# tayloraswift/swift-png

Measured on AMD Instinct MI355X. Metric: decoded_mpixels_per_s, higher is better.
Workload: dtype u8

## Files before the change

swift_png_amd/csrc/pinflate2.hip:

```cpp
#include "common.hpp"
#include <type_traits>
#include <cstddef>
#include "huffman.hpp"

namespace spng {

#ifdef SPNG_EMU
#define AS_GLOBAL
#else
#define AS_GLOBAL __attribute__((address_space(1)))
#endif
__device__ __forceinline__ uint32_t mul24(uint32_t a, uint32_t b)
{
#ifdef SPNG_EMU
    return (a & 0xffffffu) * (b & 0xffffffu);
#else
    uint32_t r;
    asm("v_mul_u32_u24 %0, %1, %2" : "=v"(r) : "v"(a), "v"(b));
    return r;
#endif
}
typedef uint32_t v4u __attribute__((vector_size(16)));
struct __attribute__((packed)) PV4 { v4u v; };
typedef uint8_t AS_GLOBAL g8;
typedef uint16_t AS_GLOBAL g16;
typedef uint32_t AS_GLOBAL g32;
typedef PV4 AS_GLOBAL gPV4;
typedef uint32_t v2u __attribute__((vector_size(8)));
struct __attribute__((packed)) PV2 { v2u v; };
typedef PV2 AS_GLOBAL gPV2;

#ifdef SPNG_NO_HINTS
#define RARE(c) (c)
#else
#define RARE(c) __builtin_expect((c), 0)
#endif
static constexpr int LB = 9, DB = 8, MB = 7;
#ifndef SPNG_SDW_MAX
#define SPNG_SDW_MAX 9
#endif
static constexpr int SDW_MAX = SPNG_SDW_MAX;
static constexpr int STAGE2_DW = SDW_MAX * 64 + 16;
static constexpr uint32_t PAGE_SHIFT = 16;
static constexpr uint32_t PAGE_UNITS = 1u << (PAGE_SHIFT - 4);
static constexpr uint64_t NONE2 = ~0ull;
static constexpr uint32_t TK_NULL = 0xffffu;

__device__ __forceinline__ uint32_t tk_m0(uint32_t run, uint32_t dist) { return 0x8000u | ((dist - 1) & 63) << 8 | (run - 3); }
__device__ __forceinline__ uint32_t tk_m1(uint32_t dist) { return 0xC000u | (dist - 1) >> 6; }

struct DPool { uint8_t *base; uint32_t *next; uint32_t pages, pad; };

#ifdef SPNG_D_PROF
#define DP_ARG , uint64_t *dp
#define DP_PASS , dp
#define DP(k) do { const uint64_t now_ = __builtin_readcyclecounter(); dp[k] += now_ - dp[31]; dp[31] = now_; } while (0)
#define DPN(k, v) (dp[k] += (v))
#define HP_ARG , uint64_t *dp = nullptr
#define HP(k) do { if (dp) DP(k); } while (0)
#else
#define DP_ARG
#define DP_PASS
#define DP(k)
#define DPN(k, v)
#define HP_ARG
#define HP(k)
#endif

#if defined(SPNG_EMU) && defined(SPNG_EMU_COV)
static long g_cov[13];
#define COV(k) __atomic_fetch_add(&g_cov[k], 1, __ATOMIC_RELAXED)
#else
#define COV(k) ((void)0)
#endif

static constexpr uint32_t EXT = 480;

enum { C_LIT = 0, C_EOB = 1, C_REF = 2, C_BAD = 3, C_LIT2 = 6, C_LINK = 7 };
__device__ __forceinline__ uint32_t lit_entry2(uint32_t sym, uint32_t len)
{
    if (sym < 256) return len | C_LIT << 5 | len << 8 | sym << 16;
    if (sym == 256) return len | C_EOB << 5 | len << 8;
    uint32_t base, cx;
    if (sym < 265) { base = sym - 254; cx = 0; }
    else if (sym < 285) { cx = (sym - 261) >> 2; base = ((4 + ((sym - 265) & 3)) << cx) + 3; }
    else if (sym == 285) { base = 258; cx = 0; }
    else { base = 0; cx = 0; }
    return (len + cx) | (base ? C_REF : C_BAD) << 5 | len << 8 | cx << 12 | base << 16;
}
__device__ __forceinline__ uint32_t dist_entry2(uint32_t sym, uint32_t len)
{
    uint32_t base, ox;
    if (sym < 4) { base = sym + 1; ox = 0; }
    else if (sym < 30) { ox = (sym >> 1) - 1; base = ((2 + (sym & 1)) << ox) + 1; }
    else { base = 0; ox = 0; }
    return (len + ox) | (base ? 0u : 32u) | len << 8 | ox << 12 | base << 16;
}
static constexpr uint32_t DIST_UNDEF = 1 | 32;

struct DLds {
    uint32_t lit[1 << LB];
    uint32_t dist[1 << DB];
    uint32_t ext[EXT];
    uint32_t stage[STAGE2_DW];
    union {
        struct {
            uint8_t  lens[512];
            uint32_t clut[1 << MB];
            uint32_t hb[6][16];
            uint32_t cl[32];
            uint16_t first[2][16];
            uint16_t codes[6][64];
        } h;
        struct {
            uint32_t ent[64];
            uint32_t vmap[SDW_MAX * 64];
            uint16_t flag[64], mpos[64];
        } c;
    };
};
static constexpr uint32_t QB = (uint32_t)offsetof(DLds, stage) * 8;
static_assert(QB % 32 == 0 && QB + (SDW_MAX * 64 + 3) * 32 + 64 < 65536, "biased positions: dword-aligned, 16 bits");
static_assert(offsetof(DLds, c.vmap) == offsetof(DLds, c.ent) + 256 && offsetof(DLds, c.flag) == offsetof(DLds, c.vmap) + SDW_MAX * 256,
              "round 1 reads ent as the row in front of vmap; round 0's empty OR behind a lane's last word lands in flag / mpos");

__device__ __forceinline__ v4u ld16(const g8 *src, uint64_t n, uint64_t off)
{
    v4u v = {0, 0, 0, 0};
    if (off + 16 <= n) v = ((const gPV4 *)(src + off))->v;
    else if (off < n) {
        uint32_t w[4] = {0, 0, 0, 0};
        for (int b = 0; b < 16; ++b) if (off + b < n) w[b >> 2] |= (uint32_t)src[off + b] << (8 * (b & 3));
        v[0] = w[0]; v[1] = w[1]; v[2] = w[2]; v[3] = w[3];
    }
    return v;
}
__device__ __forceinline__ void stage_bytes2(uint32_t *dst, const g8 *src, uint64_t n, uint64_t from, int dwords, int lane)
{
    for (int k = 0; k * 256 < dwords; ++k)
        if (k * 256 + lane * 4 < dwords) *(v4u *)(dst + k * 256 + lane * 4) = ld16(src, n, from + (uint64_t)k * 1024 + (uint64_t)lane * 16);
    WSYNC();
}
__device__ __forceinline__ void fetch2(const uint32_t *stage, uint32_t q, uint32_t &lo, uint32_t &hi)
{
    const uint32_t w = q >> 5;
    const uint32_t d0 = stage[w], d1 = stage[w + 1], d2 = stage[w + 2];
    lo = __builtin_amdgcn_alignbit(d1, d0, q);
    hi = __builtin_amdgcn_alignbit(d2, d1, q);
}
__device__ __forceinline__ uint32_t upeek32_2(const uint32_t *stage, uint32_t q)
{
    uint32_t lo, hi;
    fetch2(stage, q, lo, hi);
    return UNI(lo);
}
__device__ __forceinline__ uint64_t upeek64_2(const uint32_t *stage, uint32_t q)
{
    uint32_t lo, hi;
    fetch2(stage, q, lo, hi);
    return (uint64_t)UNI(hi) << 32 | UNI(lo);
}

struct Hdr2 {
    uint32_t type, bfinal;
    uint64_t payload;
    uint32_t stored;
    uint32_t minlen;
    uint32_t pairs;
};

template <int ROOT, int KIND>
__device__ __forceinline__ void place_symbol(uint32_t *lut, uint32_t sym, uint32_t my, uint32_t code)
{
    if (my <= (uint32_t)ROOT) lut[code << ((uint32_t)ROOT - my)] = KIND == 0 ? lit_entry2(sym, my) : dist_entry2(sym, my);
    else atomicMax(&lut[code >> (my - (uint32_t)ROOT)], my);
}
template <int ROOT, int KIND>
__device__ __forceinline__ void place_long(const uint32_t *lut, uint32_t *ext, uint32_t sym, uint32_t my, uint32_t code)
{
    if (my > (uint32_t)ROOT) {
        const uint32_t rev = __brev(code) >> (32 - my);
        const uint32_t link = lut[rev & ((1u << ROOT) - 1)];
        const uint32_t sub = (link >> 8) & 15, at = link >> 16;
        const uint32_t e = KIND == 0 ? lit_entry2(sym, my) : dist_entry2(sym, my);
        for (uint32_t j = rev >> ROOT; j < (1u << sub); j += 1u << (my - ROOT)) ext[at + j] = e;
    }
}
template <int ROOT>
__device__ __forceinline__ bool finish_root(uint32_t *lut, uint32_t &used, uint32_t cap, bool links, int lane)
{
    constexpr int PER = (1 << ROOT) / 64;
    uint32_t v[PER];
#pragma unroll
    for (int k = 0; k < PER; ++k) v[k] = lut[lane * PER + k];
#pragma unroll
    for (int k = 1; k < PER; ++k) v[k] = v[k] ? v[k] : v[k - 1];
    const unsigned long long have = __ballot(v[PER - 1] != 0) & ((1ull << lane) - 1);
    const uint32_t cin = (uint32_t)__shfl((int)v[PER - 1], have ? 63 - __clzll((long long)have) : 0, 64);
#pragma unroll
    for (int k = 0; k < PER; ++k) v[k] = v[k] ? v[k] : cin;
    if (links) {
        uint32_t need = 0;
#pragma unroll
        for (int k = 0; k < PER; ++k) need += (v[k] > (uint32_t)ROOT && v[k] <= 15) ? 1u << (v[k] - ROOT) : 0u;
        uint32_t tot;
        uint32_t at = used + wave_excl_scan(need, tot, lane);
        tot += used;
#ifdef SPNG_EMU_TRACE
        if (tot > cap && lane == 0) fprintf(stderr, "finish_root<%d>: need %u > cap %u\n", ROOT, tot, cap);
#endif
        if (tot > cap) return false;
        used = tot;
#pragma unroll
        for (int k = 0; k < PER; ++k)
            if (v[k] > (uint32_t)ROOT && v[k] <= 15) { const uint32_t sub = v[k] - ROOT; v[k] = C_LINK << 5 | sub << 8 | at << 16; at += 1u << sub; }
    }
    WSYNC();
#pragma unroll
    for (int k = 0; k < PER; ++k) lut[__brev((uint32_t)(lane * PER + k)) >> (32 - ROOT)] = v[k];
    return true;
}

__device__ __forceinline__ bool build_clut(DLds &s, uint32_t mylen, int lane)
{
    uint32_t cnt = 0, before = 0;
#pragma unroll
    for (uint32_t l = 1; l <= 7; ++l) {
        const unsigned long long m = __ballot(lane < 19 && mylen == l);
        cnt = (uint32_t)lane == l ? (uint32_t)__popcll(m) : cnt;
        before = mylen == l ? (uint32_t)__popcll(m & ((1ull << lane) - 1)) : before;
    }
    const uint32_t scaled = (lane >= 1 && lane <= 7) ? cnt << (7 - lane) : 0u;
    if (UNI(wave_sum(scaled)) != 128u) return false;
    const uint32_t first = ((row_scan(scaled) - scaled) >> (7 - (lane & 7))) & 127;
    if (lane < 16) s.h.cl[lane] = first;
    s.h.clut[lane] = 0; s.h.clut[64 + lane] = 0;
    WSYNC();
    if (lane < 19 && mylen)
        s.h.clut[(s.h.cl[mylen] + before) << (MB - mylen)] =
            mylen | (lane < 16 ? 0u : lane == 16 ? 2u : lane == 17 ? 3u : 7u) << 4 | (lane < 16 ? 1u : lane == 18 ? 11u : 3u) << 8 | (uint32_t)lane << 16;
    WSYNC();
    uint32_t none = 0;
    finish_root<MB>(s.h.clut, none, 0, false, lane);
    WSYNC();
    return true;
}

__device__ __attribute__((always_inline)) bool decode_lengths2(DLds &s, uint32_t &rel, uint32_t rel_end, uint32_t want, int lane)
{
    for (int i = lane; i < 128; i += 64) ((uint32_t *)s.h.lens)[i] = 0;
    uint32_t *list = s.lit;
    uint32_t ntok = 0, have = 0, p = rel;
    for (int window = 0; window < 80 && have < want; ++window) {
        if (p >= rel_end || p + 64 + 16 > 256u * 32) return false;
        const uint32_t q = p + (uint32_t)lane;
        const uint32_t w = q >> 5;
        const uint32_t bits = __builtin_amdgcn_alignbit(s.stage[w + 1], s.stage[w], q);
        const uint32_t e = s.h.clut[bits & ((1u << MB) - 1)];
        const uint32_t len = e & 15, sym = e >> 16, extra = (e >> 4) & 15;
        const uint32_t rep = ((e >> 8) & 0xff) + ((bits >> len) & ((1u << extra) - 1));
        const uint32_t nb = len + extra;
        uint32_t jn = nb, jr = rep;
        uint32_t jlo = lane < 32 ? 1u << lane : 0u, jhi = lane < 32 ? 0u : 1u << (lane - 32);
#pragma unroll
        for (int round = 0; round < 3; ++round) {
            const uint32_t tgt = (uint32_t)lane + jn;
            const uint32_t on = (uint32_t)__shfl((int)(jn | jr << 8), (int)(tgt & 63), 64);
            const uint32_t olo = (uint32_t)__shfl((int)jlo, (int)(tgt & 63), 64), ohi = (uint32_t)__shfl((int)jhi, (int)(tgt & 63), 64);
            if (tgt < 64) { jn += on & 0xff; jr += on >> 8; jlo |= olo; jhi |= ohi; }
        }
        unsigned long long mask = 0;
        uint32_t pp = 0;
        while (pp < 64) {
            mask |= (unsigned long long)(uint32_t)__builtin_amdgcn_readlane((int)jhi, (int)pp) << 32 | (uint32_t)__builtin_amdgcn_readlane((int)jlo, (int)pp);
            have += (uint32_t)__builtin_amdgcn_readlane((int)jr, (int)pp);
            pp += (uint32_t)__builtin_amdgcn_readlane((int)jn, (int)pp);
        }
        if ((mask >> lane) & 1) list[ntok + (uint32_t)__popcll(mask & ((1ull << lane) - 1))] = sym | rep << 8 | (q + nb) << 16;
        ntok += (uint32_t)__popcll(mask);
        p += pp;
    }
    if (have < want) return false;
    WSYNC();
    uint32_t prev = 0; bool prev_ok = false;
    have = 0;
    for (uint32_t b = 0; b < ntok; b += 64) {
        const bool is = b + (uint32_t)lane < ntok;
        const uint32_t t = is ? list[b + (uint32_t)lane] : 0u;
        const uint32_t sym = t & 0xff, r = (t >> 8) & 0xff;
        uint32_t tot;
        const uint32_t idx = have + wave_excl_scan(r, tot, lane);
        const uint32_t val = sym < 16 ? sym : 0u;
        const unsigned long long defm = __ballot(is && sym != 16);
        const unsigned long long below = defm & ((1ull << lane) - 1);
        const int pl = below ? 63 - __clzll((long long)below) : 0;
        const uint32_t pv = (uint32_t)__shfl((int)val, pl, 64);
        const uint32_t lastcur = below ? pv : prev;
        const bool ok = below ? true : prev_ok;
        const bool active = is && idx < want;
        const bool bad = active && (idx + r > want || (sym == 16 && !ok));
        if (active && !bad) {
            if (sym < 16) s.h.lens[idx] = (uint8_t)sym;
            else if (sym == 16) for (uint32_t k = 0; k < r; ++k) s.h.lens[idx + k] = (uint8_t)lastcur;
        }
        const unsigned long long endm = __ballot(active && idx + r == want);
        if (__ballot(bad)) return false;
        if (endm) {
            rel = (uint32_t)__builtin_amdgcn_readlane((int)(t >> 16), __ffsll((long long)endm) - 1);
            WSYNC();
            return rel <= rel_end;
        }
        have += tot;
        if (defm) { prev = (uint32_t)__shfl((int)val, 63 - __clzll((long long)defm), 64); prev_ok = true; }
    }
    return false;
}

__device__ __attribute__((always_inline)) bool build_tables2(DLds &s, uint32_t literals, uint32_t distances, uint32_t &minlen, uint32_t &pairs, int lane)
{
    uint32_t packed = 0;
#pragma unroll
    for (int k = 0; k < 5; ++k) { const uint32_t sym = (uint32_t)lane + 64u * k; packed |= (sym < literals ? (uint32_t)s.h.lens[sym] : 0u) << (4 * k); }
    packed |= ((uint32_t)lane < distances ? (uint32_t)s.h.lens[literals + lane] : 0u) << 20;
#define LL(k) ((packed >> (4 * (k))) & 15)
#define DL ((packed >> 20) & 15)
    for (int i = lane; i < 96; i += 64) (&s.h.hb[0][0])[i] = 0;
    WSYNC();
#pragma unroll
    for (int k = 0; k < 5; ++k) __hip_atomic_fetch_add(&s.h.hb[k][LL(k)], 1u, __ATOMIC_RELAXED, __HIP_MEMORY_SCOPE_WORKGROUP);
    __hip_atomic_fetch_add(&s.h.hb[5][DL], 1u, __ATOMIC_RELAXED, __HIP_MEMORY_SCOPE_WORKGROUP);
    const uint32_t dl = DL;
    const uint32_t dused = (uint32_t)__popcll(__ballot(dl != 0));
    const unsigned long long d1m = __ballot(dl == 1);
    WSYNC();
    const uint32_t L = (uint32_t)lane & 15;
    const bool isd = lane >= 16 && lane < 32;
    uint32_t c = 0;
// ... 8 lines not shown
    const uint32_t scaled = c << (15 - L);
    const uint32_t kraft = row_scan(scaled);
    const uint32_t klit = (uint32_t)__builtin_amdgcn_readlane((int)kraft, 15);
    const uint32_t kdist = (uint32_t)__builtin_amdgcn_readlane((int)kraft, 31);
    if (klit != 32768u) return false;
    const bool stub = dused == 0 || (dused == 1 && d1m != 0);
    if (!stub && kdist != 32768u) return false;
    if (lane < 32) s.h.first[isd ? 1 : 0][L] = (uint16_t)((kraft - scaled) >> (15 - L));
    {
        const unsigned long long nz = __ballot(lane < 16 && c != 0);
        minlen = (uint32_t)__ffsll((long long)nz) - 1;
    }
#pragma unroll
    for (int j = 0; j < (1 << LB) / 64; ++j) s.lit[j * 64 + lane] = 0;
#pragma unroll
    for (int j = 0; j < (1 << DB) / 64; ++j)
        s.dist[j * 64 + lane] = !stub ? 0u : (dused && !((j * 64 + lane) & 1)) ? dist_entry2((uint32_t)(__ffsll((long long)d1m) - 1), 1) : DIST_UNDEF;
    WSYNC();
#pragma unroll
    for (int k = 0; k < 5; ++k) {
        const uint32_t my = LL(k);
        unsigned long long same = ~0ull;
#pragma unroll
        for (int b = 0; b < 4; ++b) {
            const unsigned long long bk = __ballot((my >> b) & 1);
            same &= (my >> b) & 1 ? bk : ~bk;
        }
        if (my) {
            const uint32_t code = s.h.first[0][my] + s.h.hb[k][my] + (uint32_t)__popcll(same & ((1ull << lane) - 1));
            s.h.codes[k][lane] = (uint16_t)code;
            place_symbol<LB, 0>(s.lit, (uint32_t)lane + 64u * k, my, code);
        }
    }
    if (!stub) {
        const uint32_t my = dl;
        unsigned long long same = ~0ull;
#pragma unroll
        for (int b = 0; b < 4; ++b) {
            const unsigned long long bk = __ballot((my >> b) & 1);
            same &= (my >> b) & 1 ? bk : ~bk;
        }
        if (my) {
            const uint32_t code = s.h.first[1][my] + (uint32_t)__popcll(same & ((1ull << lane) - 1));
            s.h.codes[5][lane] = (uint16_t)code;
            place_symbol<DB, 1>(s.dist, (uint32_t)lane, my, code);
        }
    }
    WSYNC();
    const bool longl = __ballot(LL(0) > (uint32_t)LB || LL(1) > (uint32_t)LB || LL(2) > (uint32_t)LB || LL(3) > (uint32_t)LB || LL(4) > (uint32_t)LB) != 0;
    const bool longd = !stub && __ballot(dl > (uint32_t)DB) != 0;
    uint32_t used = 0;
    if (!UB(finish_root<LB>(s.lit, used, EXT, longl, lane))) return false;
    if (!stub) { if (!UB(finish_root<DB>(s.dist, used, EXT, longd, lane))) return false; }
    WSYNC();
    if (longl || longd) {
#pragma unroll
        for (int k = 0; k < 5; ++k) if (LL(k) > (uint32_t)LB) place_long<LB, 0>(s.lit, s.ext, (uint32_t)lane + 64u * k, LL(k), s.h.codes[k][lane]);
        if (!stub && dl > (uint32_t)DB) place_long<DB, 1>(s.dist, s.ext, (uint32_t)lane, dl, s.h.codes[5][lane]);
        WSYNC();
    }
#undef LL
#undef DL
    bool made = false;
    if (2 * minlen <= (uint32_t)LB)
#pragma unroll
    for (int k = 0; k < (1 << LB) / 64; ++k) {
        const uint32_t idx = (uint32_t)k * 64 + (uint32_t)lane;
        const uint32_t e = s.lit[idx];
        const uint32_t len0 = (e >> 8) & 15;
        if (((e >> 5) & 7) == C_LIT && len0 < (uint32_t)LB) {
            const uint32_t e2 = s.lit[idx >> len0];
            const uint32_t c2 = (e2 >> 5) & 7, len1 = (e2 >> 8) & 15;
            if ((c2 == C_LIT || c2 == C_LIT2) && len0 + len1 <= (uint32_t)LB) {
                s.lit[idx] = (len0 + len1) | C_LIT2 << 5 | len0 << 8 | (e & 0x00ff0000u) | (e2 & 0x00ff0000u) << 8;
                made = true;
            }
        }
    }
    pairs = __ballot(made) != 0 ? 1u : 0u;
    WSYNC();
    return true;
}

__device__ __attribute__((always_inline)) bool parse_header2(DLds &s, const g8 *src, uint64_t n, uint64_t pos, Hdr2 &h, int lane HP_ARG)
{
    const uint64_t total = n * 8;
    if (pos + 3 > total) return false;
    const uint64_t wbyte = (pos >> 5) << 2;
    stage_bytes2(s.stage, src, n, wbyte, 256, lane);
    HP(24);
    uint32_t rel = (uint32_t)(pos - wbyte * 8);
    const uint32_t first = upeek32_2(s.stage, rel);
    h.bfinal = first & 1; h.type = (first >> 1) & 3;
    h.stored = 0; h.minlen = 7; h.payload = 0; h.pairs = 0;
    if (h.type == 0) {
        const uint64_t boundary = (pos + 3 + 7) & ~(uint64_t)7;
        if (boundary + 32 > total) return false;
        const uint32_t v = upeek32_2(s.stage, (uint32_t)(boundary - wbyte * 8));
        const uint32_t l = v & 0xffff, m = v >> 16;
        if (l != (~m & 0xffffu)) return false;
        const uint64_t from = boundary / 8 + 4;
        if (from + l > n) return false;
        h.stored = l; h.payload = from * 8;
        return true;
    }
    if (h.type == 3) return false;
    uint32_t literals, distances;
    if (h.type == 1) {
        for (int i = lane; i < 320; i += 64) s.h.lens[i] = i < 144 ? 8 : i < 256 ? 9 : i < 280 ? 7 : i < 288 ? 8 : 5;
        WSYNC();
        literals = 288; distances = 32;
        h.payload = pos + 3;
    } else {
        if (pos + 17 > total) return false;
        literals = 257 + ((first >> 3) & 31);
        distances = 1 + ((first >> 8) & 31);
        const uint32_t codelengths = 4 + ((first >> 13) & 15);
        rel += 17;
        if (pos + 17 + 3 * (uint64_t)codelengths > total) return false;
        if (literals > 286) return false;
        const uint64_t packed = upeek64_2(s.stage, rel) & ((1ull << (3 * codelengths)) - 1);
        rel += 3 * codelengths;
        const uint32_t sym = (uint32_t)lane;
        const uint32_t at = sym >= 16 ? sym - 16 : sym == 0 ? 3u : sym <= 7 ? 19 - 2 * sym : 2 * sym - 12;
        const uint32_t mylen = (lane < 19 && at < codelengths) ? (uint32_t)((packed >> (3 * (at < 19 ? at : 0))) & 7) : 0u;
        if (!UB(build_clut(s, mylen, lane))) return false;
        HP(25);
        const uint32_t rel_end = (uint32_t)((total - wbyte * 8) > 0xffffffffull ? 0xffffffffu : (total - wbyte * 8));
        if (!UB(decode_lengths2(s, rel, rel_end, literals + distances, lane))) return false;
        h.payload = wbyte * 8 + rel;
        HP(26);
    }
    uint32_t minlen = 7, pairs = 0;
    if (!UB(build_tables2(s, literals, distances, minlen, pairs, lane))) return false;
    h.minlen = UNI(minlen); h.pairs = UNI(pairs);
    HP(27);
    return true;
}

static constexpr uint32_t D2_EOB = C_EOB, D2_REF = C_REF, D2_BAD = C_BAD;
template <bool FULL, bool PAIRS>
__device__ __forceinline__ uint32_t decode_at2(const DLds &s, uint32_t q, uint32_t &k, uint32_t &len0, uint32_t &h0, uint32_t &h1)
{
    uint32_t lo, hi;
    {
        const uint32_t *w = (const uint32_t *)((const uint8_t *)&s + ((q >> 3) & ~3u));
        const uint32_t d0 = w[0], d1 = w[1], d2 = w[2];
        lo = __builtin_amdgcn_alignbit(d1, d0, q);
        hi = __builtin_amdgcn_alignbit(d2, d1, q);
    }
    uint32_t e = s.lit[lo & ((1 << LB) - 1)];
    if (RARE((e & 0xe0) == 0xe0)) e = s.ext[(e >> 16) + ((lo >> LB) & ((1u << ((e >> 8) & 15)) - 1))];
    uint32_t p2 = e & 31, cls = (e >> 5) & 7;
    len0 = (e >> 8) & 15;
    uint32_t nbits = p2;
    k = cls;
    if (cls == C_REF) {
        const uint32_t b2 = __builtin_amdgcn_alignbit(hi, lo, p2);
        uint32_t d = s.dist[b2 & ((1 << DB) - 1)];
        if (RARE((d & 0x80) != 0)) d = s.ext[(d >> 16) + ((b2 >> DB) & ((1u << ((d >> 8) & 15)) - 1))];
        nbits = p2 + (d & 31);
        k |= (d >> 5) & 1;
        if (FULL) {
            const uint32_t len1 = (e >> 8) & 15, cx = (e >> 12) & 15, dl = (d >> 8) & 15, ox = (d >> 12) & 15;
            const uint32_t run = (e >> 16) + ((lo >> len1) & ((1u << cx) - 1));
            const uint32_t dd = (d >> 16) + ((b2 >> dl) & ((1u << ox) - 1));
            h0 = tk_m0(run, dd); h1 = tk_m1(dd);
        }
    } else if (FULL) {
        h0 = PAIRS ? (e >> 16) & 0xff : e >> 16; h1 = e >> 24;
    }
    return nbits;
}

template <uint32_t RETRY>
__global__ __launch_bounds__(64) void pinf2_find_kernel(const PStream *__restrict__ streams, PSeg *__restrict__ segs, uint32_t seg0)
{
    constexpr uint32_t retry = RETRY;
    __shared__ __attribute__((aligned(16))) DLds s;
    __shared__ __attribute__((aligned(16))) uint32_t win[512 + 16];
    __shared__ __attribute__((aligned(16))) uint8_t k3[512];
    const int lane = threadIdx.x;
    PSeg &sg = segs[seg0 + blockIdx.x];
    const PStream &st = streams[UNI(sg.stream)];
    if (retry && UNI(st.pass) != 1) return;
    const g8 *src = (const g8 *)uni64((uint64_t)st.src);
    const uint64_t n = uni64(st.src_len), total = n * 8;
    const uint32_t j = UNI(sg.index);
    uint64_t found = NONE2;
    const uint64_t resume_bit = uni64(st.start_bit);
    if (UNI(st.serial_only)) {
    } else if (j == 0) {
        if (resume_bit) found = resume_bit;
        else if (UNI(st.format) == SPNG_FORMAT_IOS) found = 0;
        else if (n >= 2) {
            const uint32_t cmf = src[0], flg = src[1];
            if ((cmf & 15) == 8 && (cmf >> 4) < 8 && ((cmf << 8) + flg) % 31 == 0 && !(flg & 0x20)) found = 16;
        }
    } else {
#pragma unroll
        for (int i = 0; i < 8; ++i) {
            const uint32_t x = (uint32_t)lane * 8 + i;
            const uint32_t a = x & 7, b = (x >> 3) & 7, c = x >> 6;
            k3[x] = (uint8_t)(((128u >> a) & 127) + ((128u >> b) & 127) + ((128u >> c) & 127));
        }
        const uint64_t sb = uni64(st.seg_bytes) * 8;
        const uint64_t lo_nom = uni64(st.seg_origin) * 8 + (uint64_t)j * sb;
        const uint64_t floor_bit = uni64(st.tok_bit) ? uni64(st.tok_bit) : resume_bit;
        const uint64_t lo_bit = lo_nom > floor_bit ? lo_nom : ((floor_bit + 1 + 63) & ~(uint64_t)63);
        const uint64_t hi_bit = lo_nom + sb < total ? lo_nom + sb : total;
        for (uint64_t wb = lo_bit; wb < hi_bit && found == NONE2; wb += 16384) {
            stage_bytes2(win, src, n, wb >> 3, 512, lane);
            {
                const uint64_t off = (wb >> 3) + 2048 + (uint64_t)lane * 4;
                uint32_t v = 0;
                if (lane < 16) { for (int b = 0; b < 4; ++b) if (off + b < n) v |= (uint32_t)src[off + b] << (8 * b); win[512 + lane] = v; }
                WSYNC();
            }
// ... 3 lines not shown
                const uint32_t w = ss * 64 + (uint32_t)lane, base = w * 32;
                const uint32_t d0 = win[w], d1 = win[w + 1], d2 = win[w + 2], d3 = win[w + 3];
                auto sh = [&](uint32_t k) -> uint32_t { return __builtin_amdgcn_alignbit(d1, d0, k); };
                uint32_t M = ~sh(1) & sh(2);
                M &= ~(sh(4) & sh(5) & sh(6) & sh(7));
                M &= ~(sh(9) & sh(10) & sh(11) & sh(12));
                if (base + 32 > hi_rel) M &= base >= hi_rel ? 0u : ~(~0u << (hi_rel - base));
                uint32_t R = 0;
                while (M) {
                    const uint32_t i = (uint32_t)__ffs((int)M) - 1;
                    M &= M - 1;
                    const uint32_t v0 = __builtin_amdgcn_alignbit(d1, d0, i), v1 = __builtin_amdgcn_alignbit(d2, d1, i), v2 = __builtin_amdgcn_alignbit(d3, d2, i);
                    const uint32_t ncl = ((v0 >> 13) & 15) + 4, nb = 3 * ncl;
                    if (base + i + 17 + nb > tot_rel) continue;
                    uint32_t lo = __builtin_amdgcn_alignbit(v1, v0, 17), hi = __builtin_amdgcn_alignbit(v2, v1, 17);
                    lo &= nb >= 32 ? ~0u : ~(~0u << nb);
                    hi &= nb <= 32 ? 0u : ~(~0u << (nb - 32));
                    const uint32_t kraft = (uint32_t)k3[lo & 511] + k3[(lo >> 9) & 511] + k3[(lo >> 18) & 511] +
                                           k3[__builtin_amdgcn_alignbit(hi, lo, 27) & 511] + k3[(hi >> 4) & 511] + k3[(hi >> 13) & 511] + k3[(hi >> 22) & 511];
                    R |= kraft == 128 ? 1u << i : 0u;
                }
                unsigned long long lm = __ballot(R != 0);
                while (lm && found == NONE2) {
                    const int l = __ffsll((long long)lm) - 1;
                    uint32_t r = (uint32_t)__builtin_amdgcn_readlane((int)R, l);
                    while (r && found == NONE2) {
                        const uint64_t at = wb + (ss * 64 + (uint32_t)l) * 32 + ((uint32_t)__ffs((int)r) - 1);
                        Hdr2 h;
                        if (UB(parse_header2(s, src, n, at, h, lane))) found = at;
                        r &= r - 1;
                    }
                    lm &= lm - 1;
                }
            }
        }
    }
    if (lane == 0) { sg.start_bit = found; sg.end_bit = 0; sg.ntok = 0; sg.tok_base = 0; sg.status = PSEG_FAIL; sg.used = 0; sg.next = 0; }
}

static constexpr uint32_t PAGE_HW = 1u << (PAGE_SHIFT - 1);
struct Cursor {
    uint64_t nhw;
    uint32_t npages;
    g8      *pa;
    bool     dry;
};

__device__ __forceinline__ g8 *take_page(const DPool &pool, g32 *pt, uint32_t pt_cap, Cursor &c, int lane)
{
    if (c.npages >= pt_cap) { c.dry = true; return nullptr; }
    uint32_t id = 0;
    if (lane == 0) id = atomicAdd(pool.next, 1u);
    id = UNI(id);
    if (id >= pool.pages) { c.dry = true; return nullptr; }
    if (lane == 0) pt[c.npages] = id;
    c.npages += 1;
    return (g8 *)(pool.base + ((uint64_t)id << PAGE_SHIFT));
}

__device__ __forceinline__ bool reserve_tokens(const DPool &pool, g32 *pt, uint32_t pt_cap, Cursor &c, uint32_t count, g8 *&pb, int lane)
{
    pb = c.pa;
    if (!count) return true;
    const uint64_t first_pg = c.nhw >> (PAGE_SHIFT - 1), last_pg = (c.nhw + count - 1) >> (PAGE_SHIFT - 1);
    if (first_pg == c.npages) { c.pa = take_page(pool, pt, pt_cap, c, lane); if (!c.pa) return false; }
    pb = c.pa;
    if (last_pg != first_pg) { pb = take_page(pool, pt, pt_cap, c, lane); if (!pb) return false; }
    return true;
}
__device__ __forceinline__ g16 *token_at(g8 *pa, g8 *pb, uint32_t r)
{
    return (g16 *)((r < PAGE_HW ? pa : pb) + ((uint64_t)(r & (PAGE_HW - 1)) << 1));
}
__device__ __forceinline__ void advance_tokens(Cursor &c, uint32_t count, g8 *pb)
{
    const uint64_t pg = c.nhw >> (PAGE_SHIFT - 1);
    c.nhw += count;
    if ((c.nhw >> (PAGE_SHIFT - 1)) != pg) c.pa = pb;
}

template <bool PAIRS, bool RM, bool CLAMP = false>
__device__ __forceinline__ uint32_t decode_chunk(DLds &s, const g8 *src, uint64_t n, uint64_t cb,
                                                 uint64_t entry, uint32_t sdw, const DPool &pool, g32 *pt, uint32_t pt_cap, Cursor &cur,
                                                 uint64_t &next, uint64_t &nbytes, uint64_t stop, int lane DP_ARG)
{
    DP(0);
    const uint32_t sb = sdw * 32, chb = sb * 64;
    const uint64_t sbyte = (cb >> 5) << 2;
    stage_bytes2(s.stage, src, n, sbyte, (int)((sdw * 64 + 3 + 3) & ~3u), lane);
    const uint64_t sbit = sbyte * 8;
    const uint64_t left = n * 8 - sbit;
    const uint32_t lim = left > 0xffffffffull - QB ? 0xffffffffu : (uint32_t)left + QB;
    const uint32_t off0 = (uint32_t)(cb - sbit) + QB, cend = CLAMP ? (uint32_t)(stop - sbit) + QB : off0 + chb;
    const uint32_t sub0 = off0 + (uint32_t)lane * sb, sub1 = sub0 + sb;
    const uint32_t r0end = CLAMP ? (sub1 < cend ? sub1 : cend) : sub1;
#pragma unroll
    for (int w = 0; w < SDW_MAX; ++w) s.c.vmap[w * 64 + lane] = 0;
    s.c.flag[lane] = 0;
    s.c.ent[lane] = 0;
    WSYNC();
    uint32_t d0, d1;
    if (lane == 0) COV(RM ? 2 : 3);
    DP(1);
    const uint32_t q0 = lane == 0 ? (uint32_t)(entry - sbit) + QB : sub0;
    uint32_t q = q0, st = 0;
    uint64_t mb0 = 0, mb1 = 0;
    uint32_t ntk = 0, edge = 0;
    uint32_t qx = 0;
    while (q < r0end) {
        DPN(16, 1);
        uint32_t k, len0;
        uint32_t nb = decode_at2<false, PAIRS>(s, q, k, len0, d0, d1);
        if (RARE((k & 1) != 0)) { st = k == D2_EOB ? 1u : 2u; qx = k == D2_EOB ? q + nb : q; q = 0xffffffffu; continue; }
        const uint32_t b = q - sub0;
        if (RM) {
            uint32_t m = 1;
            if (k == D2_REF) { const bool last = b + 1 == sb; m = last ? 1u : 3u; edge = last ? 1u : edge; if (last) COV(0); else if ((b & 31) == 31) COV(1); }
            const uint64_t mm = (uint64_t)m << (b & 31);
            atomicOr(&s.c.vmap[(b >> 5) * 64 + lane], (uint32_t)mm);
            atomicOr(&s.c.vmap[(b >> 5) * 64 + 64 + lane], (uint32_t)(mm >> 32));
        } else {
            atomicOr(&s.c.vmap[(b >> 5) * 64 + lane], 1u << (b & 31));
            const uint64_t bit = (uint64_t)(PAIRS ? (k == D2_REF ? 1u : 0u) : k >> 1) << (ntk & 63);
            mb0 |= ntk < 64 ? bit : 0ull; mb1 |= ntk < 64 ? 0ull : bit;
            ntk += 1;
        }
        if (PAIRS && k == C_LIT2) {
            const uint32_t b2 = b + len0;
            if (b2 < (CLAMP ? r0end - sub0 : sb)) {
                atomicOr(&s.c.vmap[(b2 >> 5) * 64 + lane], 1u << (b2 & 31));
                if (!RM) ntk += 1;
            } else { nb = len0; COV(4); }
        }
        q += nb;
    }
    if (st) q = qx;
    if (q > lim) st = 2;
    WSYNC();
    DP(2);
    uint32_t link = 64, cnt2 = 0, nh = 0;
    uint32_t x0 = 0, x1 = 0, x2 = 0, x3 = 0;
    if (st == 0) {
        uint32_t j = (uint32_t)lane, jb = sub1;
        while (q < cend) {
            DPN(17, 1);
            if (q >= jb) {
                if (nh < 4) { x3 = x2; x2 = x1; x1 = x0; x0 = q | cnt2 << 16; }
                nh += 1; j += 1; jb += sb;
            }
            const uint32_t b = q + sb - jb;
            const uint32_t *wp = s.c.ent + (b >> 5) * 64 + j;
            const uint32_t pword = RM ? wp[0] : 0u, mword = wp[64];
            uint32_t k, len0;
            const uint32_t nb = decode_at2<false, PAIRS>(s, q, k, len0, d0, d1);
            const uint32_t front = RM ? __builtin_amdgcn_alignbit(mword, pword, 31) : 0u;
            if (RM && ((mword & front) >> (b & 31)) & 1) COV(5);
            if (((mword & ~front) >> (b & 31)) & 1) { link = j; qx = q; q = 0xffffffffu; continue; }
            if (RARE((k & 1) != 0)) { st = k == D2_EOB ? 1u : 2u; qx = k == D2_EOB ? q + nb : q; q = 0xffffffffu; continue; }
            if (CLAMP && PAIRS && k == C_LIT2 && q + len0 >= cend) { cnt2 += 1; q += len0; continue; }
            cnt2 += 1 + (PAIRS ? (k >> 1) & 1 : k >> 1);
            q += nb;
        }
        if (q == 0xffffffffu) q = qx;
        if (q > lim) st = 2;
    }
    DP(3);
    bool onpath = lane == 0;
    uint32_t jump = link;
#pragma unroll
    for (int k = 0; k < 6; ++k) {
        if (onpath && jump < 64) s.c.flag[jump] = 1;
        WSYNC();
// ... 107 lines not shown
template <bool CLAMP>
__device__ __forceinline__ uint32_t cut_chunk(DLds &s, const Hdr2 &h, const g8 *src, uint64_t n, uint64_t cb, uint64_t entry, uint32_t sdw, const DPool &pool,
                                              g32 *pt, uint32_t pt_cap, Cursor &cur, uint64_t &next, uint64_t &nbytes, uint64_t stop, int lane)
{
#ifdef SPNG_D_PROF
    uint64_t dpv[32], *dp = dpv;
    for (int i = 0; i < 32; ++i) dp[i] = 0;
#endif
    if (h.minlen >= 2)
        return h.pairs ? UNI((decode_chunk<true, true, CLAMP>(s, src, n, cb, entry, sdw, pool, pt, pt_cap, cur, next, nbytes, stop, lane DP_PASS)))
                       : UNI((decode_chunk<false, true, CLAMP>(s, src, n, cb, entry, sdw, pool, pt, pt_cap, cur, next, nbytes, stop, lane DP_PASS)));
    return h.pairs ? UNI((decode_chunk<true, false, CLAMP>(s, src, n, cb, entry, sdw, pool, pt, pt_cap, cur, next, nbytes, stop, lane DP_PASS)))
                   : UNI((decode_chunk<false, false, CLAMP>(s, src, n, cb, entry, sdw, pool, pt, pt_cap, cur, next, nbytes, stop, lane DP_PASS)));
}
__device__ __forceinline__ uint32_t chunk_dwords(uint32_t minlen)
{
    uint32_t big = minlen >= 5 ? 17u : minlen == 4 ? 15u : minlen == 3 ? 11u : minlen == 2 ? 7u : 3u;
    return big > (uint32_t)SDW_MAX ? (uint32_t)SDW_MAX : big;
}

#ifndef SPNG_D_WAVES
#define SPNG_D_WAVES 4
#endif
template <uint32_t RETRY, int WHICH>
__device__ __forceinline__ void decode_segment(DLds &s, const PStream *__restrict__ streams, PSeg *__restrict__ segs,
                                               uint32_t *__restrict__ pt_slab, const DPool &pool, uint32_t seg0, PCut *__restrict__ cuts)
{
    constexpr bool CUT = WHICH == 2;
    constexpr uint32_t retry = RETRY;
    const int lane = threadIdx.x;
    PSeg &sg = segs[seg0 + blockIdx.x];
    const PStream &st = streams[UNI(sg.stream)];
    if (retry && UNI(st.pass) != 1) return;
    if (WHICH && (UNI(st.cut_on) != 0) != CUT) return;
    const uint64_t start = uni64(sg.start_bit);
    bool mid = false;
    if (start == NONE2) {
        if constexpr (!CUT) return;
        else if (!UNI(cuts[seg0 + blockIdx.x].cut)) return;
        mid = true;
    }
    const g8 *src = (const g8 *)uni64((uint64_t)st.src);
    const uint64_t n = uni64(st.src_len);
    uint64_t limit = NONE2;
    uint32_t nk = UNI(sg.index) + 1;
    const uint32_t seg_first = UNI(st.seg_first), seg_count = UNI(st.seg_count);
    auto advance = [&](uint64_t from) {
        limit = NONE2;
        for (; nk < seg_count; ++nk) {
            const uint64_t v = uni64(segs[seg_first + nk].start_bit);
            if (v != NONE2 && v >= from) { limit = v; break; }
        }
    };
    const uint64_t segbits = CUT ? uni64(st.seg_bytes) * 8 : 0;
    const uint64_t org = CUT ? uni64(st.seg_origin) * 8 : 0;
    uint64_t guess = CUT ? org + (uint64_t)UNI(sg.index) * segbits : 0;
    const uint64_t tok0 = CUT && UNI(sg.index) == 0 ? uni64(st.tok_bit) : 0;
    bool inside = tok0 != 0;
    advance(CUT && mid ? guess + 1 : start + 1);
    g32 *pt = (g32 *)(pt_slab + uni64(sg.log_off));
    uint32_t pt_cap;
    {
        const PSeg &upto = segs[seg_first + (nk < seg_count ? nk : seg_count - 1)];
        const uint64_t end = uni64(upto.log_off) + (nk < seg_count ? 0 : uni64(upto.log_cap));
        const uint64_t room = end - uni64(sg.log_off);
        pt_cap = room > 0xffffff00ull ? 0xffffff00u : (uint32_t)room;
    }
    uint32_t tgt = UNI(sg.index) + 1;
    if (CUT && tgt < seg_count && UNI(cuts[seg_first + tgt].cut)) {
        const uint64_t room = uni64(sg.log_cap);
        pt_cap = room > 0xffffff00ull ? 0xffffff00u : (uint32_t)room;
    }
    uint32_t nrec = 0, slides = 0;
    bool fresh = true, stopped = false;
    uint64_t tbl = 0, tbl_id = 0, head_tbl = 0;
    bool tbl_here = false;
    Cursor cur;
    cur.nhw = 0; cur.npages = 0; cur.pa = nullptr; cur.dry = false;
    uint64_t pos = start;
    int32_t status = PSEG_FAIL;
    const bool resumable = uni64((uint64_t)st.state) != 0;
    uint64_t hw_block = 0, nbytes = 0, bytes_block = 0;
    uint32_t nblocks = 0;
#ifdef SPNG_D_PROF
    uint64_t dp[32];
    for (int i = 0; i < 32; ++i) dp[i] = 0;
    dp[31] = __builtin_readcyclecounter();
    const uint64_t dp_t0 = dp[31];
#endif
    if (CUT && mid) pos = uni64(segs[seg_first + UNI(cuts[seg0 + blockIdx.x].anchor)].start_bit);
    for (;;) {
        if (!(CUT && mid) && pos >= limit) {
            if (pos == limit) { status = PSEG_CONT; break; }
            nk += 1; advance(pos);
            continue;
        }
        Hdr2 h;
        hw_block = cur.nhw; bytes_block = nbytes;
        DP(7);
        const bool hok_ = UB(parse_header2(s, src, n, pos, h, lane DP_PASS));
        DP(8);
        DPN(23, 1);
#ifdef SPNG_EMU_TRACE
        if (!hok_ && lane == 0) fprintf(stderr, "header at bit %llu rejected\n", (unsigned long long)pos);
#endif
        if (!hok_) break;
        if (CUT && (mid || inside) && h.type == 0) break;
        if (h.type == 0) {
            const uint64_t from = h.payload / 8;
            bool ok = true;
            for (uint32_t k = 0; k < h.stored && ok; k += PAGE_HW / 2) {
                const uint32_t m = h.stored - k < PAGE_HW / 2 ? h.stored - k : PAGE_HW / 2;
                g8 *pb;
                ok = UB(reserve_tokens(pool, pt, pt_cap, cur, m, pb, lane));
                if (ok) {
                    const uint32_t r0 = (uint32_t)(cur.nhw & (PAGE_HW - 1));
                    for (uint32_t i = (uint32_t)lane; i < m; i += 64) *token_at(cur.pa, pb, r0 + i) = (uint16_t)src[from + k + i];
                    advance_tokens(cur, m, pb);
                    nbytes += m;
                }
            }
            if (!ok) break;
            pos = h.payload + (uint64_t)h.stored * 8;
        } else if constexpr (CUT) {
            const uint32_t sdw = chunk_dwords(h.minlen);
            const uint64_t chb = (uint64_t)sdw * 32 * 64;
            const uint64_t id = table_id(h, pos);
            if (mid) head_tbl = id;
            uint64_t entry = mid ? guess : inside ? tok0 : h.payload, cb = entry;
            uint32_t state = 0;
            for (;;) {
                uint64_t stop_at = NONE2;
                for (; tgt < seg_count && UNI(cuts[seg_first + tgt].cut); ++tgt) {
                    const uint64_t v = org + (uint64_t)tgt * segbits + chb;
                    if (v > cb) { stop_at = v; break; }
                }
                const bool last = stop_at != NONE2 && cb + chb >= stop_at;
                uint64_t next;
                if (last || (mid && nrec < PCUT_RECS))
                    state = cut_chunk<true>(s, h, src, n, cb, entry, sdw, pool, pt, pt_cap, cur, next, nbytes, last ? stop_at : cb + chb, lane);
                else
                    state = cut_chunk<false>(s, h, src, n, cb, entry, sdw, pool, pt, pt_cap, cur, next, nbytes, 0, lane);
                entry = uni64(next);
                if (mid && fresh && state) {
                    if (cur.dry || ++slides > CUT_SLIDES || cb + chb >= n * 8) { state = 2; break; }
                    COV(6);
                    guess = cb + chb; entry = cb = guess;
                    continue;
                }
                fresh = false;
                if (mid && nrec < PCUT_RECS && !state) {
                    const uint32_t padn = (8 - (uint32_t)(cur.nhw & 7)) & 7;
                    g8 *pb;
                    if (!UB(reserve_tokens(pool, pt, pt_cap, cur, padn, pb, lane))) { state = 2; break; }
                    if (padn) {
                        const uint32_t r0 = (uint32_t)(cur.nhw & (PAGE_HW - 1));
                        if ((uint32_t)lane < padn) *token_at(cur.pa, pb, r0 + (uint32_t)lane) = (uint16_t)TK_NULL;
                        advance_tokens(cur, padn, pb);
                    }
                    if (lane == 0) { PCut &ct = cuts[seg0 + blockIdx.x]; ct.rec[nrec].bit = entry; ct.rec[nrec].hw = (uint32_t)cur.nhw; ct.rec[nrec].bytes = (uint32_t)nbytes; }
                    nrec += 1;
                }
                if (last && !state) { stopped = true; break; }
                if (state) break;
                cb += chb;
            }
            if (stopped) { status = PSEG_CUT; tbl = pos; tbl_id = id; tbl_here = !(mid || inside); pos = entry; break; }
            if (state != 1) break;
            pos = entry;
            mid = false; inside = false;
        } else {
            uint32_t big = h.minlen >= 5 ? 17u : h.minlen == 4 ? 15u : h.minlen == 3 ? 11u : h.minlen == 2 ? 7u : 3u;
            if (big > (uint32_t)SDW_MAX) big = (uint32_t)SDW_MAX;
            uint32_t sdw = big < 9u ? big : 9u;
            uint64_t entry = h.payload, cb = h.payload;
            uint32_t state = 0;
            for (;;) {
                uint64_t next;
                if (h.minlen >= 2)
                    state = h.pairs ? UNI((decode_chunk<true, true>(s, src, n, cb, entry, sdw, pool, pt, pt_cap, cur, next, nbytes, 0, lane DP_PASS)))
                                    : UNI((decode_chunk<false, true>(s, src, n, cb, entry, sdw, pool, pt, pt_cap, cur, next, nbytes, 0, lane DP_PASS)));
                else
                    state = h.pairs ? UNI((decode_chunk<true, false>(s, src, n, cb, entry, sdw, pool, pt, pt_cap, cur, next, nbytes, 0, lane DP_PASS)))
                                    : UNI((decode_chunk<false, false>(s, src, n, cb, entry, sdw, pool, pt, pt_cap, cur, next, nbytes, 0, lane DP_PASS)));
                entry = uni64(next);
                if (state) break;
                cb += (uint64_t)sdw * 32 * 64;
                sdw = big;
            }
            if (state != 1) break;
            pos = entry;
        }
        nblocks += 1;
        if (h.bfinal) { status = PSEG_FINAL; break; }
    }
    if (lane == 0 && nblocks) atomicAdd(pool.next + 1, nblocks);
    uint64_t nhw = cur.nhw;
    if (status == PSEG_FAIL && cur.dry && !retry) status = PSEG_NOPAGE;
    else if (status == PSEG_FAIL && resumable && !(CUT && (mid || inside))) { status = PSEG_PARTIAL; nhw = hw_block; nbytes = bytes_block; }
    if (lane == 0) { sg.end_bit = pos; sg.ntok = nhw; sg.nbytes = nbytes; sg.status = status; sg.next = CUT && stopped ? tgt : nk; }
    if (retry && lane == 0) sg.head = 0;
    if (CUT && lane == 0) { PCut &ct = cuts[seg0 + blockIdx.x]; ct.tbl = tbl; ct.tbl_id = tbl_id; ct.nrec = nrec; ct.head_tbl = head_tbl; ct.tbl_here = tbl_here ? 1u : 0u; ct.tbl_bytes = bytes_block; }
#ifdef SPNG_D_PROF
    if (blockIdx.x == 1 && lane == 0)
        printf("decode: %lu blocks %lu chunks %lu halfwords %lu windows; lane-0 steps r0 %lu r1 %lu replay %lu; cycles: total %lu stage %lu setup %lu round0 %lu "
               "round1 %lu path %lu replay %lu flush %lu header %lu (stage %lu clut %lu lengths %lu tables %lu) other %lu\n",
               dp[23], dp[20], dp[21], dp[22], dp[16], dp[17], dp[18], __builtin_readcyclecounter() - dp_t0, dp[0], dp[1], dp[2], dp[3], dp[4], dp[5], dp[6], dp[8] + dp[24] + dp[25] + dp[26] + dp[27], dp[24], dp[25], dp[26], dp[27], dp[7]);
#endif
}

template <uint32_t RETRY>
__global__ __launch_bounds__(64, SPNG_D_WAVES) void pinf2_decode_kernel(const PStream *__restrict__ streams, PSeg *__restrict__ segs,
                                                          uint32_t *__restrict__ pt_slab, DPool pool, uint32_t seg0)
{
    __shared__ __attribute__((aligned(16))) DLds s;
    decode_segment<RETRY, 0>(s, streams, segs, pt_slab, pool, seg0, nullptr);
}
template <int WHICH>
__global__ __launch_bounds__(64, SPNG_D_WAVES) void pinf2_cutdecode_kernel(const PStream *__restrict__ streams, PSeg *__restrict__ segs,
                                                             uint32_t *__restrict__ pt_slab, DPool pool, uint32_t seg0, PCut *__restrict__ cuts)
{
    __shared__ __attribute__((aligned(16))) DLds s;
    decode_segment<0, WHICH>(s, streams, segs, pt_slab, pool, seg0, cuts);
}

__device__ __forceinline__ bool back_to_the_header(PStream &st, PSeg *__restrict__ segs, int lane)
{
    const bool deep = uni64(st.tok_bit) - uni64(st.start_bit) > RESUME_SERIAL_BITS;
    if (deep) {
        const uint32_t first = UNI(st.seg_first), count = UNI(st.seg_count);
        for (uint32_t i = (uint32_t)lane; i < count; i += 64) segs[first + i].start_bit = NONE2;
    }
    if (lane == 0) {
        if (deep) st.serial_only = 1;
        else { st.tok_bit = 0; st.out_pos = st.blk_out; }
    }
    __threadfence();
    return !deep;
}

__global__ __launch_bounds__(64) void pinf2_cutplan_kernel(PStream *__restrict__ streams, PSeg *__restrict__ segs, PCut *__restrict__ cuts, uint32_t *__restrict__ stats)
{
    __shared__ __attribute__((aligned(16))) DLds s;
    const int lane = threadIdx.x;
    PStream &st = streams[blockIdx.x];
    const uint32_t need = UNI(st.cut_segs);
    if (!need || UNI(st.serial_only)) return;
    const uint32_t first = UNI(st.seg_first), count = UNI(st.seg_count);
    const g8 *src = (const g8 *)uni64((uint64_t)st.src);
    const uint64_t n = uni64(st.src_len), sb = uni64(st.seg_bytes), org = uni64(st.seg_origin);
    const bool rcut = UNI(st.cut_resumed) != 0;
    {
        uint32_t prev = ~0u;
        for (uint32_t base = 0; base < count; base += 64) {
            const uint32_t i = base + (uint32_t)lane;
            unsigned long long mask = __ballot(i < count && segs[first + i].start_bit != NONE2);
            while (mask) {
                const uint32_t f = base + (uint32_t)__ffsll((long long)mask) - 1;
                mask &= mask - 1;
                bool keep = true;
                if (prev != ~0u && f - prev - 1 >= need) {
                    const uint64_t at = uni64(segs[first + f].start_bit);
                    Hdr2 h;
                    if (UB(parse_header2(s, src, n, uni64(segs[first + prev].start_bit), h, lane)) && h.type != 0) {
                        uint32_t len = 0, code = 0;
                        for (uint32_t k = 0; k < (1u << LB) / 64; ++k) {
                            const uint32_t idx = k * 64 + (uint32_t)lane, e = s.lit[idx];
                            const unsigned long long m = __ballot(((e >> 5) & 7) == C_EOB);
                            if (m && !len) {
                                const int l = __ffsll((long long)m) - 1;
                                len = (uint32_t)__shfl((int)((e >> 8) & 15), l, 64);
                                code = (k * 64 + (uint32_t)l) & ((1u << len) - 1);
                            }
// ... 811 lines not shown
```

Baseline: 35740.

## Prefetch first chunk during table build and reuse staged bytes for next header

While building the Huffman tables for a dynamic block, the decoder now issues global loads for the first decode chunk into registers and writes them to the LDS stage afterwards, so the first chunk skips its own staging. It also remembers the last staged window and reuses it when parsing the next block header, restaging only if the code-length decode runs off the end of the window. Both aim to hide or avoid global-memory load latency on the serial per-block path. In exchange they add register pressure for the prefetch buffer and a retry path for header parsing.

Result: no change. 35680 (-0.2%).

```diff
diff --git a/swift_png_amd/csrc/pinflate2.hip b/swift_png_amd/csrc/pinflate2.hip
--- a/swift_png_amd/csrc/pinflate2.hip
+++ b/swift_png_amd/csrc/pinflate2.hip
@@ -68,7 +68,7 @@
 #endif
 
 #if defined(SPNG_EMU) && defined(SPNG_EMU_COV)
-static long g_cov[13];
+static long g_cov[15];
 #define COV(k) __atomic_fetch_add(&g_cov[k], 1, __ATOMIC_RELAXED)
 #else
 #define COV(k) ((void)0)
@@ -167,7 +167,11 @@
     uint32_t stored;
     uint32_t minlen;
     uint32_t pairs;
+    uint32_t staged;
 };
+static constexpr int PRE_SDW = SDW_MAX < 9 ? SDW_MAX : 9;
+static constexpr int PRE_DW = (PRE_SDW * 64 + 3 + 3) & ~3;
+static_assert(PRE_DW <= STAGE2_DW, "the first chunk's bytes fit the stage");
 
 template <int ROOT, int KIND>
 __device__ __forceinline__ void place_symbol(uint32_t *lut, uint32_t sym, uint32_t my, uint32_t code)
@@ -246,13 +250,14 @@
     return true;
 }
 
-__device__ __attribute__((always_inline)) bool decode_lengths2(DLds &s, uint32_t &rel, uint32_t rel_end, uint32_t want, int lane)
+__device__ __attribute__((always_inline)) bool decode_lengths2(DLds &s, uint32_t &rel, uint32_t rel_end, uint32_t want, uint32_t stage_bits, bool &ranoff, int lane)
 {
     for (int i = lane; i < 128; i += 64) ((uint32_t *)s.h.lens)[i] = 0;
     uint32_t *list = s.lit;
     uint32_t ntok = 0, have = 0, p = rel;
     for (int window = 0; window < 80 && have < want; ++window) {
-        if (p >= rel_end || p + 64 + 16 > 256u * 32) return false;
+        if (p >= rel_end) return false;
+        if (p + 64 + 16 > stage_bits) { ranoff = true; return false; }
         const uint32_t q = p + (uint32_t)lane;
         const uint32_t w = q >> 5;
         const uint32_t bits = __builtin_amdgcn_alignbit(s.stage[w + 1], s.stage[w], q);
@@ -427,17 +432,23 @@
     return true;
 }
 
-__device__ __attribute__((always_inline)) bool parse_header2(DLds &s, const g8 *src, uint64_t n, uint64_t pos, Hdr2 &h, int lane HP_ARG)
+template <bool PRE = false>
+__device__ __attribute__((always_inline)) bool parse_header2(DLds &s, const g8 *src, uint64_t n, uint64_t pos, Hdr2 &h, int lane,
+                                                             uint64_t have_byte = NONE2, uint32_t have_dw = 0 HP_ARG)
 {
     const uint64_t total = n * 8;
     if (pos + 3 > total) return false;
-    const uint64_t wbyte = (pos >> 5) << 2;
-    stage_bytes2(s.stage, src, n, wbyte, 256, lane);
+    const uint64_t own = (pos >> 5) << 2;
+    const bool kept = have_byte != NONE2 && own >= have_byte && own + 16 <= have_byte + (uint64_t)have_dw * 4;
+    uint64_t wbyte = kept ? have_byte : own;
+    uint32_t stage_bits = kept ? have_dw * 32 : 256u * 32;
+    if (!kept) stage_bytes2(s.stage, src, n, wbyte, 256, lane);
+    else if (lane == 0) COV(14);
     HP(24);
     uint32_t rel = (uint32_t)(pos - wbyte * 8);
     const uint32_t first = upeek32_2(s.stage, rel);
     h.bfinal = first & 1; h.type = (first >> 1) & 3;
-    h.stored = 0; h.minlen = 7; h.payload = 0; h.pairs = 0;
+    h.stored = 0; h.minlen = 7; h.payload = 0; h.pairs = 0; h.staged = 0;
     if (h.type == 0) {
         const uint64_t boundary = (pos + 3 + 7) & ~(uint64_t)7;
         if (boundary + 32 > total) return false;
@@ -471,14 +482,37 @@
         const uint32_t mylen = (lane < 19 && at < codelengths) ? (uint32_t)((packed >> (3 * (at < 19 ? at : 0))) & 7) : 0u;
         if (!UB(build_clut(s, mylen, lane))) return false;
         HP(25);
-        const uint32_t rel_end = (uint32_t)((total - wbyte * 8) > 0xffffffffull ? 0xffffffffu : (total - wbyte * 8));
-        if (!UB(decode_lengths2(s, rel, rel_end, literals + distances, lane))) return false;
+        for (bool again = kept;; again = false) {
+            const uint32_t rel_end = (uint32_t)((total - wbyte * 8) > 0xffffffffull ? 0xffffffffu : (total - wbyte * 8));
+            bool ranoff = false;
+            if (UB(decode_lengths2(s, rel, rel_end, literals + distances, stage_bits, ranoff, lane))) break;
+            if (!again || !UB(ranoff)) return false;
+            if (lane == 0) COV(13);
+            wbyte = own; stage_bits = 256u * 32;
+            stage_bytes2(s.stage, src, n, wbyte, 256, lane);
+            rel = (uint32_t)(pos - wbyte * 8) + 17 + 3 * codelengths;
+        }
         h.payload = wbyte * 8 + rel;
         HP(26);
+    }
+    v4u pre[(PRE_DW + 255) / 256];
+    const uint64_t pbyte = (h.payload >> 5) << 2;
+    const bool ask = PRE && h.type == 2;
+    if (ask) {
+#pragma unroll
+        for (int k = 0; k * 256 < PRE_DW; ++k)
+            if (k * 256 + lane * 4 < PRE_DW) pre[k] = ld16(src, n, pbyte + (uint64_t)k * 1024 + (uint64_t)lane * 16);
     }
     uint32_t minlen = 7, pairs = 0;
     if (!UB(build_tables2(s, literals, distances, minlen, pairs, lane))) return false;
     h.minlen = UNI(minlen); h.pairs = UNI(pairs);
+    if (ask) {
+#pragma unroll
+        for (int k = 0; k * 256 < PRE_DW; ++k)
+            if (k * 256 + lane * 4 < PRE_DW) *(v4u *)(s.stage + k * 256 + lane * 4) = pre[k];
+        WSYNC();
+        h.staged = PRE_DW;
+    }
     HP(27);
     return true;
 }
@@ -648,12 +682,12 @@
 template <bool PAIRS, bool RM, bool CLAMP = false>
 __device__ __forceinline__ uint32_t decode_chunk(DLds &s, const g8 *src, uint64_t n, uint64_t cb,
                                                  uint64_t entry, uint32_t sdw, const DPool &pool, g32 *pt, uint32_t pt_cap, Cursor &cur,
-                                                 uint64_t &next, uint64_t &nbytes, uint64_t stop, int lane DP_ARG)
+                                                 uint64_t &next, uint64_t &nbytes, uint64_t stop, int lane DP_ARG, bool staged = false)
 {
     DP(0);
     const uint32_t sb = sdw * 32, chb = sb * 64;
     const uint64_t sbyte = (cb >> 5) << 2;
-    stage_bytes2(s.stage, src, n, sbyte, (int)((sdw * 64 + 3 + 3) & ~3u), lane);
+    if (!staged) stage_bytes2(s.stage, src, n, sbyte, (int)((sdw * 64 + 3 + 3) & ~3u), lane);
     const uint64_t sbit = sbyte * 8;
     const uint64_t left = n * 8 - sbit;
     const uint32_t lim = left > 0xffffffffull - QB ? 0xffffffffu : (uint32_t)left + QB;
@@ -927,6 +961,8 @@
     const bool resumable = uni64((uint64_t)st.state) != 0;
     uint64_t hw_block = 0, nbytes = 0, bytes_block = 0;
     uint32_t nblocks = 0;
+    uint64_t have_byte = NONE2;
+    uint32_t have_dw = 0;
 #ifdef SPNG_D_PROF
     uint64_t dp[32];
     for (int i = 0; i < 32; ++i) dp[i] = 0;
@@ -943,7 +979,13 @@
         Hdr2 h;
         hw_block = cur.nhw; bytes_block = nbytes;
         DP(7);
-        const bool hok_ = UB(parse_header2(s, src, n, pos, h, lane DP_PASS));
+#ifdef SPNG_NO_PRESTAGE
+        constexpr bool PRE = false;
+#else
+        constexpr bool PRE = !CUT;
+#endif
+        const bool hok_ = UB(parse_header2<PRE>(s, src, n, pos, h, lane, have_byte, have_dw DP_PASS));
+        have_byte = NONE2;
         DP(8);
         DPN(23, 1);
 #ifdef SPNG_EMU_TRACE
@@ -1020,20 +1062,24 @@
             uint32_t sdw = big < 9u ? big : 9u;
             uint64_t entry = h.payload, cb = h.payload;
             uint32_t state = 0;
+            bool there = h.staged != 0;
             for (;;) {
                 uint64_t next;
                 if (h.minlen >= 2)
-                    state = h.pairs ? UNI((decode_chunk<true, true>(s, src, n, cb, entry, sdw, pool, pt, pt_cap, cur, next, nbytes, 0, lane DP_PASS)))
-                                    : UNI((decode_chunk<false, true>(s, src, n, cb, entry, sdw, pool, pt, pt_cap, cur, next, nbytes, 0, lane DP_PASS)));
+                    state = h.pairs ? UNI((decode_chunk<true, true>(s, src, n, cb, entry, sdw, pool, pt, pt_cap, cur, next, nbytes, 0, lane DP_PASS, there)))
+                                    : UNI((decode_chunk<false, true>(s, src, n, cb, entry, sdw, pool, pt, pt_cap, cur, next, nbytes, 0, lane DP_PASS, there)));
                 else
-                    state = h.pairs ? UNI((decode_chunk<true, false>(s, src, n, cb, entry, sdw, pool, pt, pt_cap, cur, next, nbytes, 0, lane DP_PASS)))
-                                    : UNI((decode_chunk<false, false>(s, src, n, cb, entry, sdw, pool, pt, pt_cap, cur, next, nbytes, 0, lane DP_PASS)));
+                    state = h.pairs ? UNI((decode_chunk<true, false>(s, src, n, cb, entry, sdw, pool, pt, pt_cap, cur, next, nbytes, 0, lane DP_PASS, there)))
+                                    : UNI((decode_chunk<false, false>(s, src, n, cb, entry, sdw, pool, pt, pt_cap, cur, next, nbytes, 0, lane DP_PASS, there)));
                 entry = uni64(next);
                 if (state) break;
                 cb += (uint64_t)sdw * 32 * 64;
                 sdw = big;
+                there = false;
             }
             if (state != 1) break;
+            have_byte = (cb >> 5) << 2;
+            have_dw = there ? h.staged : (sdw * 64 + 3 + 3) & ~3u;
             pos = entry;
         }
         nblocks += 1;
```
